# surrealdb/surrealdb

Measured on AMD Instinct MI355X. Metric: knn_qps, higher is better.
Workload: dtype f32; 1 GPU; brute-force cosine KNN, 10000000 rows/GPU x 768-dim f32, K=10, single query (BASELINE configs[1]); batch=0, rows_total=10000000, rows_per_gpu=10000000, dim=768, k=10, distance=cosine, parallelism=single

## Files before the change

surrealdb_amd/csrc/sdbv.hip:

```cpp

#include <hip/hip_runtime.h>
#include <rocblas/rocblas.h>

#include <algorithm>
#include <atomic>
#include <cfloat>
#include <chrono>
#include <cmath>
#include <cstdint>
#include <deque>
#include <limits>
#include <memory>
#include <thread>
#include <unordered_set>
#include <cstdio>
#include <cstring>
#include <map>
#include <mutex>
#include <queue>
#include <set>
#include <string>
#include <unordered_map>
#include <vector>

// ... 17 lines not shown
struct Shadow {
	int kind = 0;
	bool h4 = false;
	void *codes = nullptr;
	float *side = nullptr;
	uint64_t sn_pad = 0;
	uint64_t bytes = 0;
	float *pinv() const { return side; }
	float *pscale() const { return side; }
	float *peps() const { return side + sn_pad; }
	float *l2_xx() const { return side + sn_pad; }
	float *l2_res() const { return side + 2 * sn_pad; }
	uint32_t *xsum() const { return (uint32_t *)(side + 2 * sn_pad); }
	float *peps4() const { return h4 ? side + 3 * sn_pad : nullptr; }
	uint32_t *xsum_h() const {
		return h4 ? (uint32_t *)(side + 4 * sn_pad) : nullptr;
	}
	uint32_t *plane_h() const { return (uint32_t *)codes; }
	uint32_t *plane_l(uint32_t d) const {
		return plane_h() + (uint64_t)((d + 31) / 32) * sn_pad * 4;
	}
};

struct Table {
	uint64_t n = 0;
	uint64_t n_pad = 0;
	uint32_t d = 0;
	uint8_t metric = 0;
	double order = 0.0;
	float *cm = nullptr;
	double *norms = nullptr;
	float *aux = nullptr;
	uint32_t *bunc = nullptr;
	uint32_t bunc_n = 0;
	double bmax_norm = 0.0;
	uint64_t *ids_dev = nullptr;
	Shadow sh;
	uint64_t bytes = 0;
};

struct sdbv_ctx {
	int device = 0;
	hipStream_t stream = nullptr;
	std::map<uint64_t, Table> tables;
	std::mutex mu;
	std::string err;
	sdbv_stats stats{};
	void *block_out = nullptr;
	uint64_t block_out_cap = 0;
	void *final_out = nullptr;
	void *merge_tmp = nullptr;
	float *q_dev = nullptr;
	float *q_pin = nullptr;
	uint32_t q_cap = 0;
	hipEvent_t ev0, ev1, ev2, ev3, ev4;
	float *pf_scores = nullptr;
	uint64_t pf_scores_cap = 0;
	uint32_t *pf_rows = nullptr;
	uint32_t *pf4_list = nullptr;
	void *pf4_thr = nullptr;
	void *pf_cands = nullptr;
	void *pf_res = nullptr;
	uint64_t pf_slots[2][6] = {};
	rocblas_handle blas = nullptr;
	float *S = nullptr;
	uint64_t S_cap = 0;
	void *bstate = nullptr;
	uint64_t bstate_cap = 0;
	float *Q_dev = nullptr;
	uint64_t Q_cap = 0;
	double *qnorms = nullptr;
	uint64_t qnorms_cap = 0;
	double *bdists = nullptr;
	uint64_t bdists_cap = 0;
	uint32_t *btheta = nullptr;
	uint64_t btheta_cap = 0;
	void *bcand = nullptr;
	uint64_t bcand_cap = 0;
	uint32_t *bcand_cnt = nullptr;
	uint64_t bcand_cnt_cap = 0;
	double ms_gemm = 0, ms_select = 0, ms_exact = 0;
	uint64_t *flt_mask = nullptr;
	uint64_t *flt_mask_pin = nullptr;
	uint64_t flt_mask_cap = 0;
	uint32_t *flt_rows = nullptr;
	uint32_t *flt_rows_pin = nullptr;
	void *flt_cands = nullptr;
};

struct Cand {
	double dist;
	uint64_t id;
};

__device__ __host__ static inline uint64_t d_splitmix64(uint64_t z) {
	z += 0x9E3779B97F4A7C15ULL;
	z = (z ^ (z >> 30)) * 0xBF58476D1CE4E5B9ULL;
	z = (z ^ (z >> 27)) * 0x94D049BB133111EBULL;
	return z ^ (z >> 31);
}

__device__ __host__ static inline float d_gen_elem(uint64_t seed, uint64_t gidx) {
	uint64_t x = d_splitmix64(seed + gidx);
	double u = (double)(x >> 11) * 0x1.0p-53;
	return (float)(-20.0 + 40.0 * u);
}

__device__ static inline uint64_t d_total_key(double x) {
	uint64_t bits = __double_as_longlong(x);
	return (bits >> 63) ? ~bits : (bits | 0x8000000000000000ULL);
}


__global__ void k_gen_cm(float *cm, uint64_t n, uint64_t n_pad, uint32_t d,
                         uint64_t seed, uint64_t row_offset) {
	uint64_t total = (uint64_t)d * n_pad;
	for (uint64_t idx = (uint64_t)blockIdx.x * blockDim.x + threadIdx.x;
	     idx < total; idx += (uint64_t)gridDim.x * blockDim.x) {
		uint64_t k = idx / n_pad;
		uint64_t r = idx % n_pad;
		float v = 0.0f;
		if (r < n)
			v = d_gen_elem(seed, (row_offset + r) * (uint64_t)d + k);
		cm[idx] = v;
	}
}

__global__ void k_transpose(const float *__restrict__ rm, float *__restrict__ cm,
                            uint64_t n, uint64_t n_pad, uint32_t d) {
	__shared__ float tile[32][33];
	uint64_t rb = (uint64_t)blockIdx.x * 32;
	uint32_t kb = blockIdx.y * 32;
	uint32_t tx = threadIdx.x & 31, ty = threadIdx.x >> 5;
	for (uint32_t yy = ty; yy < 32; yy += 8) {
		uint64_t r = rb + yy;
		uint32_t k = kb + tx;
		tile[yy][tx] = (r < n && k < d) ? rm[r * d + k] : 0.0f;
	}
	__syncthreads();
	for (uint32_t yy = ty; yy < 32; yy += 8) {
		uint32_t k = kb + yy;
		uint64_t r = rb + tx;
		if (k < d && r < n_pad)
			cm[(uint64_t)k * n_pad + r] = tile[tx][yy];
	}
}

__global__ void k_norms(const float *__restrict__ cm, double *__restrict__ norms,
                        uint64_t n, uint64_t n_pad, uint32_t d) {
	uint64_t r = (uint64_t)blockIdx.x * blockDim.x + threadIdx.x;
	if (r >= n)
		return;
	float p[8] = {0, 0, 0, 0, 0, 0, 0, 0};
	uint32_t k = 0;
	for (; k + 8 <= d; k += 8) {
#pragma unroll
		for (uint32_t j = 0; j < 8; j++) {
			float x = cm[(uint64_t)(k + j) * n_pad + r];
			p[j] = __fadd_rn(p[j], __fmul_rn(x, x));
		}
	}
	float acc = 0.0f;
	acc = __fadd_rn(acc, __fadd_rn(__fadd_rn(p[0], p[4]), __fadd_rn(p[1], p[5])));
// ... 204 lines not shown
					acc.y = __fadd_rn(acc.y, __fmul_rn(dy, dy));
					acc.z = __fadd_rn(acc.z, __fmul_rn(dz, dz));
					acc.w = __fadd_rn(acc.w, __fmul_rn(dw, dw));
				}
				const float s[4] = {acc.x, acc.y, acc.z, acc.w};
#pragma unroll
				for (int c = 0; c < ROWS_PER_LANE; c++)
					dist[c] = sqrt((double)s[c]);
			}
		}

		uint64_t kk_key = kth_key;
		uint32_t kk_row = kth_row;
		int full = (topk_n >= (int)k);
#pragma unroll
		for (int c = 0; c < ROWS_PER_LANE; c++) {
			if (!valid[c])
				continue;
			uint64_t key = d_total_key(dist[c]);
			uint32_t row32 = (uint32_t)(r0 + c);
			bool take = !full || key < kk_key || (key == kk_key && row32 < kk_row);
			if (take) {
				int idx = atomicAdd(&cnt, 1);
				buf[idx].key = key;
				buf[idx].dist = dist[c];
				buf[idx].row = row32;
			}
		}
		__syncthreads();

		if (cnt > 0) {
			int m = cnt;
			for (int i = threadIdx.x; i < topk_n; i += THREADS)
				buf[m + i] = topk[i];
			int total = m + topk_n;
			__syncthreads();
			int new_n;
			block_select_topk(buf, total, topk, (int)k, &new_n);
			if (threadIdx.x == 0) {
				topk_n = new_n;
				if (new_n >= (int)k) {
					kth_key = topk[k - 1].key;
					kth_row = topk[k - 1].row;
				}
				cnt = 0;
			}
		}
		__syncthreads();
	}

	scan_topk_write(topk, topk_n, k, ids, block_out);
}

__device__ __forceinline__ static void merge_slice(
    Cand *__restrict__ block_out, uint64_t total, uint32_t k,
    uint64_t per_block, Cand *__restrict__ out) {
	__shared__ uint64_t red_key[THREADS / 64];
	__shared__ uint64_t red_id[THREADS / 64];
	__shared__ long red_idx[THREADS / 64];
	const int lane = threadIdx.x & 63;
	const int wave = threadIdx.x >> 6;
	const uint64_t s0 = (uint64_t)blockIdx.x * per_block;
	const uint64_t s1 = s0 + per_block < total ? s0 + per_block : total;
	out += (uint64_t)blockIdx.x * k;
	if (s0 >= total) {
		for (uint32_t i = threadIdx.x; i < k; i += THREADS) {
			out[i].dist = __longlong_as_double(0x7FF0000000000000LL);
			out[i].id = ~0ULL;
		}
		return;
	}
	for (int slot = 0; slot < (int)k; slot++) {
		uint64_t bk = ~0ULL;
		uint64_t bid = ~0ULL;
		long bi = -1;
		for (uint64_t i = s0 + threadIdx.x; i < s1; i += THREADS) {
			uint64_t ck = d_total_key(block_out[i].dist);
			uint64_t cid = block_out[i].id;
			if (ck < bk || (ck == bk && cid < bid)) {
				bk = ck;
				bid = cid;
				bi = (long)i;
			}
		}
		for (int off = 32; off > 0; off >>= 1) {
			uint64_t ok = __shfl_down(bk, off);
			uint64_t oid = __shfl_down(bid, off);
			long oi = __shfl_down(bi, off);
			if (ok < bk || (ok == bk && oid < bid)) {
				bk = ok;
				bid = oid;
				bi = oi;
			}
		}
		if (lane == 0) {
			red_key[wave] = bk;
			red_id[wave] = bid;
			red_idx[wave] = bi;
		}
		__syncthreads();
		if (threadIdx.x == 0) {
			uint64_t bbk = ~0ULL, bbid = ~0ULL;
			long best = -1;
			for (int w = 0; w < THREADS / 64; w++) {
				if (red_idx[w] < 0)
					continue;
				if (red_key[w] < bbk ||
				    (red_key[w] == bbk && red_id[w] < bbid)) {
					bbk = red_key[w];
					bbid = red_id[w];
					best = red_idx[w];
				}
			}
			if (best < 0) {
				out[slot].dist =
				    __longlong_as_double(0x7FF0000000000000LL);
				out[slot].id = ~0ULL;
			} else {
				out[slot] = block_out[best];
				block_out[best].dist =
				    __longlong_as_double(0x7FF0000000000000LL);
				block_out[best].id = ~0ULL;
// ... 881 lines not shown
			const int32_t N =
			    H4 ? (int32_t)(8u * (256u * ah2 + 16u * ah1 + ah0) -
			                   16384u * xsum[r] + qbias)
			       : PF6_N(xsum[r], qbias);
			const float pe = peps[r];
			const float a = PF6_A(
			    N, H4 ? __fmul_rn(pscale[r], 0.5f) : pscale[r], qscale);
			const float e = PF6_E(pe, qeps);
			const bool ok = allowed && r < row_end &&
			                (__float_as_uint(a) & 0x7F800000u) != 0x7F800000u;
			if constexpr (MASKED)
				scores[r] = ok        ? __fsub_rn(a, e)
				            : allowed ? ninf
				                      : __uint_as_float(0x7FC00000u);
			else
				scores[r] = ok ? __fsub_rn(a, e) : ninf;
			if (ok) {
				const uint64_t v =
				    ((uint64_t)d_key32(__fadd_rn(a, e)) << 32) | (uint32_t)r;
				if (!full || v < kthv) {
					int idx = atomicAdd(&cnt, 1);
					buf[idx] = v;
				}
			}
		}
		pf_topk_fold(buf, topk, cnt, topk_n, kth, k);
	}

	pf_topk_write(topk, topk_n, k, block_out);
}

__global__ void k_pf_compact(const float *__restrict__ scores, uint64_t n,
                             const Cand *__restrict__ approx_top, uint32_t k,
                             float eps, uint32_t *__restrict__ cand_cnt,
                             uint32_t *__restrict__ cand_rows) {
	const double thr = approx_top[k - 1].dist + 2.0 * (double)eps;
	const uint64_t ngrp = (n + 3) / 4;
	for (uint64_t g = (uint64_t)blockIdx.x * blockDim.x + threadIdx.x;
	     g < ngrp; g += (uint64_t)gridDim.x * blockDim.x) {
		const float4 s = *(const float4 *)(scores + g * 4);
		const float v[4] = {s.x, s.y, s.z, s.w};
#pragma unroll
		for (int c = 0; c < 4; c++) {
			uint64_t r = g * 4 + c;
			if (r < n && (double)v[c] <= thr) {
				uint32_t idx = atomicAdd(cand_cnt, 1u);
				if (idx < PF_CAND_CAP)
					cand_rows[idx] = (uint32_t)r;
			}
		}
	}
}

template <int METRIC>
__device__ __forceinline__ static void rows_exact_one(
    const float *__restrict__ cm, const double *__restrict__ norms,
    const uint64_t *__restrict__ ids, uint64_t n_pad, uint32_t d,
    double q_norm, uint32_t r, Cand *__restrict__ out, float *qs, float *xs,
    float *ps) {
	__syncthreads();
	for (uint32_t i = threadIdx.x; i < d; i += 64)
		xs[i] = cm[(uint64_t)i * n_pad + r];
	__syncthreads();
	if (METRIC == 0) {
		const uint32_t d8 = d & ~7u;
		if (threadIdx.x < 8) {
			float pj = 0.f;
			for (uint32_t i = threadIdx.x; i < d8; i += 8)
				pj = __fadd_rn(pj, __fmul_rn(xs[i], qs[i]));
			ps[threadIdx.x] = pj;
		}
		__syncthreads();
		if (threadIdx.x == 0) {
			float p[8];
#pragma unroll
			for (int j = 0; j < 8; j++)
				p[j] = ps[j];
			uint32_t k8 = d8;
			float sum = 0.f;
			sum = __fadd_rn(sum, __fadd_rn(p[0], p[4]));
			sum = __fadd_rn(sum, __fadd_rn(p[1], p[5]));
			sum = __fadd_rn(sum, __fadd_rn(p[2], p[6]));
			sum = __fadd_rn(sum, __fadd_rn(p[3], p[7]));
			for (; k8 < d; k8++)
				sum = __fadd_rn(sum, __fmul_rn(xs[k8], qs[k8]));
			double den = q_norm * norms[r];
			Cand o;
			o.dist = 1.0 - (double)sum / den;
			o.id = ids[r];
			*out = o;
		}
	} else {
		if (threadIdx.x == 0) {
			float acc = 0.f;
			for (uint32_t kk = 0; kk < d; kk++) {
				float diff = xs[kk] - qs[kk];
				acc = __fadd_rn(acc, __fmul_rn(diff, diff));
			}
			Cand o;
			o.dist = sqrt((double)acc);
			o.id = ids[r];
			*out = o;
		}
	}
}

template <int METRIC>
__device__ __forceinline__ static void rows_exact(
    const float *__restrict__ cm, const double *__restrict__ norms,
    const uint64_t *__restrict__ ids, uint64_t n_pad, uint32_t d,
    const float *__restrict__ qg, double q_norm,
    const uint32_t *__restrict__ rows, uint32_t cnt, Cand *__restrict__ out,
    float *qs, float *xs, float *ps) {
	for (uint32_t i = threadIdx.x; i < d; i += 64)
		qs[i] = qg[i];
	for (uint32_t c = blockIdx.x; c < cnt; c += gridDim.x)
		rows_exact_one<METRIC>(cm, norms, ids, n_pad, d, q_norm, rows[c],
		                       out + c, qs, xs, ps);
}

template <int METRIC>
__global__ __launch_bounds__(64) void k_pf_rescore(
    const float *__restrict__ cm, const double *__restrict__ norms,
    const uint64_t *__restrict__ ids, uint64_t n_pad, uint32_t d,
    const float *__restrict__ qg, double q_norm,
    const uint32_t *__restrict__ cand_cnt,
    const uint32_t *__restrict__ cand_rows, Cand *__restrict__ out) {
	__shared__ float qs[MAX_D];
	__shared__ float xs[MAX_D];
	__shared__ float ps[8];
	const uint32_t cnt = *cand_cnt;
	if (cnt > PF_CAND_CAP || blockIdx.x >= cnt)
		return;
	rows_exact<METRIC>(cm, norms, ids, n_pad, d, qg, q_norm, cand_rows, cnt,
	                   out, qs, xs, ps);
}

template <int METRIC>
__global__ __launch_bounds__(64) void k_rows_exact(
    const float *__restrict__ cm, const double *__restrict__ norms,
    const uint64_t *__restrict__ ids, uint64_t n_pad, uint32_t d,
    const float *__restrict__ qg, double q_norm,
    const uint32_t *__restrict__ rows, uint32_t cnt, Cand *__restrict__ out) {
	__shared__ float qs[MAX_D];
	__shared__ float xs[MAX_D];
	__shared__ float ps[8];
	rows_exact<METRIC>(cm, norms, ids, n_pad, d, qg, q_norm, rows, cnt, out,
	                   qs, xs, ps);
}

__global__ __launch_bounds__(THREADS) void k_pf_final(
    Cand *__restrict__ cands, const uint32_t *__restrict__ cand_cnt,
    uint32_t k, Cand *__restrict__ out) {
	const uint32_t raw = *cand_cnt;
	const uint64_t total = raw > PF_CAND_CAP ? 0 : raw;
	if (threadIdx.x == 0) {
		out[k].dist = 0.0;
		out[k].id = raw;
	}
	merge_slice(cands, total, k, total, out);
}

#define PF4_LIST_CAP 262144u
#define PF4_BLOCK_LIST 8192
#define PF4_PASSES 4
#ifndef PF4_REFINE_LANES
#define PF4_REFINE_LANES 32
#endif

__global__ __launch_bounds__(64) void k_pf4_threshold(
    const float *__restrict__ cm, const double *__restrict__ norms,
    const uint64_t *__restrict__ ids, uint64_t n_pad, uint32_t d,
    const float *__restrict__ qg, double q_norm,
    const Cand *__restrict__ approx_top, Cand *__restrict__ out) {
	__shared__ float qs[MAX_D];
	__shared__ float xs[MAX_D];
	__shared__ float ps[8];
	const uint64_t r = approx_top[blockIdx.x].id;
	if (r == ~0ULL) {
		if (threadIdx.x == 0) {
			Cand o;
			o.dist = __longlong_as_double(0x7FF0000000000000LL);
			o.id = ~0ULL;
			out[blockIdx.x] = o;
		}
		return;
	}
	for (uint32_t i = threadIdx.x; i < d; i += 64)
		qs[i] = qg[i];
	rows_exact_one<0>(cm, norms, ids, n_pad, d, q_norm, (uint32_t)r,
	                  out + blockIdx.x, qs, xs, ps);
}

__device__ __forceinline__ static double pf4_threshold(
    const Cand *__restrict__ thr, uint32_t k, unsigned long long *key) {
	if (threadIdx.x == 0)
		*key = 0;
	__syncthreads();
	if (threadIdx.x < k)
		atomicMax(key, (unsigned long long)d_total_key(thr[threadIdx.x].dist));
	__syncthreads();
	const uint64_t kb = *key;
	return __longlong_as_double(
	    (long long)((kb >> 63) ? (kb & 0x7FFFFFFFFFFFFFFFULL) : ~kb));
}

__global__ __launch_bounds__(THREADS) void k_pf4_compact(
    const float *__restrict__ scores, uint64_t n,
    const Cand *__restrict__ thr, uint32_t k, uint32_t list_cap,
    uint32_t *__restrict__ list_cnt, uint32_t *__restrict__ list_rows) {
	__shared__ uint32_t rows[PF4_BLOCK_LIST];
	__shared__ uint32_t cnt, base;
	__shared__ unsigned long long tkey;
	if (threadIdx.x == 0)
		cnt = 0;
	const double T = pf4_threshold(thr, k, &tkey);
	const uint64_t ngrp = (n + 3) / 4;
	const uint64_t round = (uint64_t)THREADS * PF4_PASSES;
	for (uint64_t g0 = (uint64_t)blockIdx.x * round;;
	     g0 += (uint64_t)gridDim.x * round) {
		const bool last = g0 >= ngrp;
		float4 s[PF4_PASSES];
#pragma unroll
		for (int p = 0; p < PF4_PASSES; p++) {
			const uint64_t g = g0 + (uint64_t)p * THREADS + threadIdx.x;
			if (g < ngrp)
				s[p] = *(const float4 *)(scores + g * 4);
		}
#pragma unroll
		for (int p = 0; p < PF4_PASSES; p++) {
			const uint64_t g = g0 + (uint64_t)p * THREADS + threadIdx.x;
			if (g >= ngrp)
				continue;
			const float v[4] = {s[p].x, s[p].y, s[p].z, s[p].w};
#pragma unroll
			for (int c = 0; c < 4; c++) {
				const uint64_t r = g * 4 + c;
				if (r < n && !((double)v[c] > T))
					rows[atomicAdd(&cnt, 1u)] = (uint32_t)r;
			}
		}
		__syncthreads();
		const uint32_t m = cnt;
		__syncthreads();
		if (m > PF4_BLOCK_LIST - 4 * THREADS * PF4_PASSES || (last && m > 0)) {
			if (threadIdx.x == 0) {
				base = atomicAdd(list_cnt, m);
				cnt = 0;
			}
			__syncthreads();
			for (uint32_t i = threadIdx.x; i < m; i += THREADS)
				if (base + i < list_cap)
					list_rows[base + i] = rows[i];
			__syncthreads();
		}
		if (last)
			break;
	}
}

__global__ __launch_bounds__(THREADS) void k_pf4_refine(
    const uint4 *__restrict__ hp, const uint2 *__restrict__ lp,
    const float *__restrict__ pscale, const float *__restrict__ peps,
    const uint32_t *__restrict__ xsum, uint64_t sn_pad, uint32_t ngroups,
    const uint32_t *__restrict__ qd, float qscale, float qeps, uint32_t qbias,
    const Cand *__restrict__ thr, uint32_t k, uint32_t list_cap,
    const uint32_t *__restrict__ list_cnt,
    const uint32_t *__restrict__ list_rows, uint32_t *__restrict__ cand_cnt,
    uint32_t *__restrict__ cand_rows) {
	__shared__ unsigned long long tkey;
	const double T = pf4_threshold(thr, k, &tkey);
	const uint32_t m = *list_cnt;
	if (m > list_cap)
		return;
	const uint32_t sub = threadIdx.x % PF4_REFINE_LANES;
	const uint32_t per_grid = gridDim.x * (THREADS / PF4_REFINE_LANES);
	for (uint32_t c = (blockIdx.x * THREADS + threadIdx.x) / PF4_REFINE_LANES;
	     c < m; c += per_grid) {
		const uint32_t r = list_rows[c];
		uint32_t ah2 = 0, ah1 = 0, ah0 = 0, al2 = 0, al1 = 0, al0 = 0;
		for (uint32_t g = sub; g < ngroups; g += PF4_REFINE_LANES) {
			const uint4 hv = hp[(uint64_t)g * sn_pad + r];
			const uint2 lv = lp[(uint64_t)g * sn_pad + r];
			PF6_GROUP(hv, lv, g)
		}
#pragma unroll
		for (int off = PF4_REFINE_LANES / 2; off > 0; off >>= 1) {
			ah2 += __shfl_xor(ah2, off);
			ah1 += __shfl_xor(ah1, off);
			ah0 += __shfl_xor(ah0, off);
			al2 += __shfl_xor(al2, off);
			al1 += __shfl_xor(al1, off);
			al0 += __shfl_xor(al0, off);
		}
		if (sub == 0) {
			const int32_t N = PF6_N(xsum[r], qbias);
			const float pe = peps[r];
			const float a = PF6_A(N, pscale[r], qscale);
			const float e = PF6_E(pe, qeps);
			const bool covered =
			    (__float_as_uint(a) & 0x7F800000u) != 0x7F800000u;
			if (!covered || !((double)__fsub_rn(a, e) > T)) {
				const uint32_t idx = atomicAdd(cand_cnt, 1u);
				if (idx < PF_CAND_CAP)
					cand_rows[idx] = r;
			}
		}
	}
}
#undef PF6_E
#undef PF6_A
#undef PF6_N
#undef PF6_GROUP
#undef PF6_GROUP_H
#undef PF6_DOT3

template <int METRIC>
__global__ void k_all_dists(const float *__restrict__ cm,
                            const double *__restrict__ norms, uint64_t n,
                            uint64_t n_pad, uint32_t d,
                            const float *__restrict__ qg, double q_norm,
                            double order, double q_mean,
                            double *__restrict__ out) {
	uint64_t r = (uint64_t)blockIdx.x * blockDim.x + threadIdx.x;
	if (r >= n)
		return;
	if (METRIC == 0) {
		float p[8] = {0, 0, 0, 0, 0, 0, 0, 0};
		uint32_t k = 0;
		for (; k + 8 <= d; k += 8) {
#pragma unroll
			for (uint32_t j = 0; j < 8; j++) {
				float x = cm[(uint64_t)(k + j) * n_pad + r];
				p[j] = __fadd_rn(p[j], __fmul_rn(x, qg[k + j]));
			}
		}
		float sum = 0.f;
		sum = __fadd_rn(sum, __fadd_rn(p[0], p[4]));
		sum = __fadd_rn(sum, __fadd_rn(p[1], p[5]));
		sum = __fadd_rn(sum, __fadd_rn(p[2], p[6]));
		sum = __fadd_rn(sum, __fadd_rn(p[3], p[7]));
		for (; k < d; k++)
			sum = __fadd_rn(sum, __fmul_rn(cm[(uint64_t)k * n_pad + r], qg[k]));
		out[r] = 1.0 - (double)sum / (q_norm * norms[r]);
	} else if (METRIC == 1) {
		float acc = 0.f;
		for (uint32_t k = 0; k < d; k++) {
			float diff = cm[(uint64_t)k * n_pad + r] - qg[k];
			acc = __fadd_rn(acc, __fmul_rn(diff, diff));
		}
		out[r] = sqrt((double)acc);
	} else if (METRIC == 2) {
		float acc = 0.f;
		for (uint32_t k = 0; k < d; k++)
			acc = __fadd_rn(acc, fabsf(qg[k] - cm[(uint64_t)k * n_pad + r]));
		out[r] = (double)acc;
	} else if (METRIC == 3) {
		float m = 0.f;
		for (uint32_t k = 0; k < d; k++)
			m = fmaxf(m, fabsf(qg[k] - cm[(uint64_t)k * n_pad + r]));
// ... 1093 lines not shown
		(void)hipFree(t.norms);
	if (t.aux)
		(void)hipFree(t.aux);
	if (t.bunc)
		(void)hipFree(t.bunc);
	if (t.ids_dev)
		(void)hipFree(t.ids_dev);
	if (t.sh.codes)
		(void)hipFree(t.sh.codes);
	if (t.sh.side)
		(void)hipFree(t.sh.side);
	t = Table{};
}

extern "C" {

int sdbv_init(int device, sdbv_ctx **out) {
	auto *ctx = new sdbv_ctx();
	if (device >= 0) {
		if (hipSetDevice(device) != hipSuccess) {
			delete ctx;
			return SDBV_ERR_HIP;
		}
		ctx->device = device;
	} else {
		(void)hipGetDevice(&ctx->device);
	}
	if (hipStreamCreate(&ctx->stream) != hipSuccess) {
		delete ctx;
		return SDBV_ERR_HIP;
	}
	(void)hipEventCreate(&ctx->ev0);
	(void)hipEventCreate(&ctx->ev1);
	(void)hipEventCreate(&ctx->ev2);
	(void)hipEventCreate(&ctx->ev3);
	(void)hipEventCreate(&ctx->ev4);
	*out = ctx;
	return SDBV_OK;
}

void sdbv_shutdown(sdbv_ctx *ctx) {
	if (!ctx)
		return;
	for (auto &kv : ctx->tables)
		free_table(kv.second);
	if (ctx->block_out)
		(void)hipFree(ctx->block_out);
	if (ctx->final_out)
		(void)hipFree(ctx->final_out);
	if (ctx->merge_tmp)
		(void)hipFree(ctx->merge_tmp);
	if (ctx->q_dev)
		(void)hipFree(ctx->q_dev);
	for (void *p : {(void *)ctx->pf_scores, (void *)ctx->pf_rows,
	                ctx->pf_cands, ctx->pf_res, (void *)ctx->pf4_list,
	                ctx->pf4_thr})
		if (p)
			(void)hipFree(p);
	for (void *p : {(void *)ctx->S, ctx->bstate, (void *)ctx->Q_dev,
	                (void *)ctx->qnorms, (void *)ctx->bdists,
	                (void *)ctx->btheta, (void *)ctx->bcand,
	                (void *)ctx->bcand_cnt})
		if (p)
			(void)hipFree(p);
	for (void *p : {(void *)ctx->flt_mask, (void *)ctx->flt_rows,
	                ctx->flt_cands})
		if (p)
			(void)hipFree(p);
	if (ctx->flt_mask_pin)
		(void)hipHostFree(ctx->flt_mask_pin);
	if (ctx->flt_rows_pin)
		(void)hipHostFree(ctx->flt_rows_pin);
	if (ctx->blas)
		(void)rocblas_destroy_handle(ctx->blas);
	(void)hipEventDestroy(ctx->ev0);
	(void)hipEventDestroy(ctx->ev1);
	(void)hipEventDestroy(ctx->ev2);
	(void)hipEventDestroy(ctx->ev3);
	(void)hipEventDestroy(ctx->ev4);
	(void)hipStreamDestroy(ctx->stream);
	delete ctx;
}

const char *sdbv_last_error(sdbv_ctx *ctx) { return ctx ? ctx->err.c_str() : ""; }

int sdbv_get_stats(sdbv_ctx *ctx, sdbv_stats *out) {
	if (!ctx || !out)
		return SDBV_ERR_BAD_ARG;
	*out = ctx->stats;
	return SDBV_OK;
}

static int stage_common(sdbv_ctx *ctx, uint64_t table, uint64_t n, uint32_t d,
                        uint8_t metric, Table **out) {
	if (d == 0 || d > MAX_D || (d % 4) != 0)
		return SDBV_ERR_BAD_ARG;
	if (metric > SDBV_METRIC_PEARSON)
		return SDBV_ERR_UNSUPPORTED;
	if (metric == SDBV_METRIC_JACCARD && d > 1024)
		return SDBV_ERR_UNSUPPORTED;
	auto it = ctx->tables.find(table);
	if (it != ctx->tables.end()) {
		free_table(it->second);
		ctx->tables.erase(it);
	}
	Table t;
// ... 413 lines not shown
	hipLaunchKernelGGL(k_fill_ids, dim3((uint32_t)nb), dim3(THREADS), 0,
	                   ctx->stream, t->ids_dev, t->n_pad, id_base);
	return finish_stage(ctx, t, true);
}

uint64_t sdbv_table_rows(sdbv_ctx *ctx, uint64_t table) {
	std::lock_guard<std::mutex> lk(ctx->mu);
	auto it = ctx->tables.find(table);
	return it == ctx->tables.end() ? 0 : it->second.n;
}

int sdbv_drop_table(sdbv_ctx *ctx, uint64_t table) {
	std::lock_guard<std::mutex> lk(ctx->mu);
	auto it = ctx->tables.find(table);
	if (it == ctx->tables.end())
		return SDBV_ERR_NO_TABLE;
	free_table(it->second);
	ctx->tables.erase(it);
	refresh_bytes_staged(ctx);
	return SDBV_OK;
}

int sdbv_table_set_order(sdbv_ctx *ctx, uint64_t table, double order) {
	std::lock_guard<std::mutex> lk(ctx->mu);
	auto it = ctx->tables.find(table);
	if (it == ctx->tables.end())
		return SDBV_ERR_NO_TABLE;
	it->second.order = order;
	return SDBV_OK;
}

static int ensure_query_scratch(sdbv_ctx *ctx, uint32_t d, uint64_t nblocks,
                                uint32_t k) {
	if (ctx->q_cap < d) {
		if (ctx->q_dev)
			(void)hipFree(ctx->q_dev);
		const size_t qb = d * sizeof(float) +
		                  (size_t)((d + 31) / 32) * PF6_QWORDS * sizeof(uint32_t);
		HIP_CHECK(ctx, hipMalloc(&ctx->q_dev, qb));
		if (ctx->q_pin)
			(void)hipHostFree(ctx->q_pin);
		HIP_CHECK(ctx, hipHostMalloc(&ctx->q_pin, qb));
		ctx->q_cap = d;
	}
	uint64_t need = nblocks * k * sizeof(Cand);
	if (ctx->block_out_cap < need) {
		if (ctx->block_out)
			(void)hipFree(ctx->block_out);
		HIP_CHECK(ctx, hipMalloc(&ctx->block_out, need));
		ctx->block_out_cap = need;
	}
	if (!ctx->final_out)
		HIP_CHECK(ctx, hipMalloc(&ctx->final_out, MAX_K * sizeof(Cand)));
	if (!ctx->merge_tmp)
		HIP_CHECK(ctx,
		          hipMalloc(&ctx->merge_tmp, 32 * MAX_K * sizeof(Cand)));
	return SDBV_OK;
}

static int stage_query(sdbv_ctx *ctx, const float *q, uint32_t d,
                       size_t q_bytes) {
	std::memcpy(ctx->q_pin, q, d * sizeof(float));
	HIP_CHECK(ctx, hipMemcpyAsync(ctx->q_dev, ctx->q_pin, q_bytes,
	                              hipMemcpyHostToDevice, ctx->stream));
	return SDBV_OK;
}

static void copy_results(const Cand *host_out, uint32_t m, uint64_t *out_ids,
                         double *out_dists, uint32_t *out_n) {
	*out_n = m;
	for (uint32_t i = 0; i < m; i++) {
		out_ids[i] = host_out[i].id;
		out_dists[i] = host_out[i].dist;
	}
}

static uint64_t scan_grid(uint64_t n, uint64_t *rows_per_block) {
	uint64_t tiles = (n + TILE - 1) / TILE;
	uint64_t nblocks = tiles < 2048 ? tiles : 2048;
	if (nblocks == 0)
		nblocks = 1;
	uint64_t tiles_per_block = (tiles + nblocks - 1) / nblocks;
	*rows_per_block = tiles_per_block * TILE;
	return (n + *rows_per_block - 1) / *rows_per_block;
}

static void launch_scan(sdbv_ctx *ctx, Table &t, uint32_t k, double q_norm,
                        uint64_t nblocks, uint64_t rows_per_block,
                        const uint64_t *mask) {
#define LAUNCH_SCAN(M, MASKED)                                                 \
	hipLaunchKernelGGL((k_scan<M, MASKED>), dim3((uint32_t)nblocks),           \
	                   dim3(THREADS), 0, ctx->stream, t.cm, t.norms, t.n,      \
	                   t.n_pad, t.d, ctx->q_dev, q_norm, k, rows_per_block,    \
	                   (Cand *)ctx->block_out, t.ids_dev, mask)
	const bool cosine = t.metric == SDBV_METRIC_COSINE;
	if (mask) {
		if (cosine)
			LAUNCH_SCAN(0, true);
		else
			LAUNCH_SCAN(1, true);
	} else {
		if (cosine)
			LAUNCH_SCAN(0, false);
		else
			LAUNCH_SCAN(1, false);
	}
// ... 430 lines not shown
	ctx->stats.last_scan_kernel_ms = ms_scan;
	ctx->stats.last_merge_kernel_ms = ms_merge;
	ctx->stats.last_rows_scanned = t.n;
	return SDBV_OK;
}

int sdbv_knn_bruteforce(sdbv_ctx *ctx, uint64_t table, const float *q,
                        uint32_t d, uint32_t k, uint64_t *out_ids,
                        double *out_dists, uint32_t *out_n) {
	std::lock_guard<std::mutex> lk(ctx->mu);
	auto it = ctx->tables.find(table);
	if (it == ctx->tables.end())
		return SDBV_ERR_NO_TABLE;
	Table &t = it->second;
	if (d != t.d)
		return SDBV_ERR_BAD_ARG;
	if (k == 0 || k > (1u << 22))
		return SDBV_ERR_BAD_ARG;
	ctx->stats.last_scan_path = 0;
	ctx->stats.last_prefilter_candidates = 0;
	ctx->stats.last_prefilter_stage1 = 0;
	if (k > MAX_K || t.metric > SDBV_METRIC_EUCLIDEAN)
		return knn_large_k(ctx, t, q, d, k, nullptr, out_ids, out_dists,
		                   out_n);

	uint64_t rows_per_block = 0;
	const uint64_t nblocks = scan_grid(t.n, &rows_per_block);
	const int kind = shadow_kind(t);
	const bool use_h4 = kind == 3 && t.sh.h4 && h4_policy(&t);
	uint64_t pf_rows_per_block = 0;
	uint64_t scratch_blocks = std::max(
	    nblocks,
	    kind ? prefilter_grid(ctx, t.n, kind, false, &pf_rows_per_block) : 0);
	if (use_h4)
		scratch_blocks = std::max(
		    scratch_blocks,
		    prefilter_grid(ctx, t.n, 4, false, &pf_rows_per_block));
	int rc = ensure_query_scratch(ctx, d, scratch_blocks, k);
	if (rc != SDBV_OK)
		return rc;
	double q_norm = sqrt((double)h_sumsq_f32(q, d));
	PfL2Q l2q;
	const bool use_pf =
	    kind == 5 ? pf_l2_query(q, d, &l2q)
	              : kind != 0 && q_norm >= PF_NORM_MIN && q_norm <= PF_NORM_MAX;
	PfQ6 q6;
	float qbias = 0.f;
	rc = stage_query_pf(ctx, q, d, q_norm, use_pf ? kind : 0, &q6, &qbias,
	                    &l2q);
	if (rc != SDBV_OK)
		return rc;

	auto t_start = std::chrono::steady_clock::now();
	Cand host_out[MAX_K + 2];
	bool served = false;
	if (use_pf && use_h4) {
		const uint32_t list_cap = pf4_list_max();
		uint32_t ncand = 0, nstage1 = 0;
		rc = knn_prefilter_h4(ctx, t, k, q_norm, q6, list_cap, host_out,
		                      &ncand, &nstage1);
		if (rc != SDBV_OK)
			return rc;
		ctx->stats.last_prefilter_stage1 = nstage1;
		if (nstage1 <= list_cap) {
			served = true;
			ctx->stats.last_prefilter_candidates = ncand;
			ctx->stats.last_scan_path = ncand <= PF_CAND_CAP ? 15u : 16u;
		}
	}
	if (use_pf && !served) {
		uint32_t ncand = 0;
		rc = knn_prefilter(ctx, t, k, q_norm, qbias, q6, nullptr, host_out,
		                   &ncand);
		if (rc != SDBV_OK)
			return rc;
		ctx->stats.last_prefilter_candidates = ncand;
		ctx->stats.last_scan_path = (ncand <= PF_CAND_CAP ? 1u : 2u) +
		                            (kind == 5 ? 16u : 2u * (uint32_t)(kind - 1));
	}
	if (!(ctx->stats.last_scan_path & 1u)) {
		rc = knn_exact_scan(ctx, t, k, q_norm, nblocks, rows_per_block,
		                    host_out);
		if (rc != SDBV_OK)
			return rc;
	}
	ctx->stats.last_total_ms =
	    std::chrono::duration<double, std::milli>(
	        std::chrono::steady_clock::now() - t_start)
	        .count();

	copy_results(host_out, (uint32_t)(k < t.n ? k : t.n), out_ids, out_dists,
	             out_n);
	return SDBV_OK;
}


uint64_t sdbv_filter_rows(const uint64_t *allow, uint64_t allow_words,
                          uint64_t n, uint32_t *out_rows, uint64_t cap) {
	if (!allow)
		return 0;
	uint64_t words = (n + 63) / 64;
	if (words > allow_words)
		words = allow_words;
	if (!out_rows)
		cap = 0;
	uint64_t count = 0;
	for (uint64_t w = 0; w < words; w++) {
// ... 122 lines not shown
	if (!allow || allow_words != (t.n + 63) / 64)
		return SDBV_ERR_BAD_ARG;
	auto t_start = std::chrono::steady_clock::now();
	const bool device_topk = k <= MAX_K && t.metric <= SDBV_METRIC_EUCLIDEAN;
	const uint64_t list_max = device_topk ? filter_rowlist_max() : 0;
	if (list_max && !ctx->flt_rows_pin)
		HIP_CHECK(ctx, hipHostMalloc(&ctx->flt_rows_pin,
		                             PF_CAND_CAP * sizeof(uint32_t)));
	const uint64_t count = sdbv_filter_rows(allow, allow_words, t.n,
	                                        ctx->flt_rows_pin, list_max);
	ctx->stats.last_scan_path = 0;
	ctx->stats.last_prefilter_candidates = 0;
	ctx->stats.last_prefilter_stage1 = 0;
	ctx->stats.last_filter_rows = count;
	ctx->stats.last_rows_scanned = count;
	ctx->stats.last_scan_kernel_ms = 0;
	ctx->stats.last_merge_kernel_ms = 0;
	ctx->stats.last_total_ms = 0;
	if (count == 0) {
		*out_n = 0;
		return SDBV_OK;
	}
	if (!device_topk)
		return knn_large_k(ctx, t, q, d, k, allow, out_ids, out_dists, out_n);

	const bool by_list = count <= list_max;
	double q_norm = sqrt((double)h_sumsq_f32(q, d));
	const int kind = shadow_kind(t);
	PfL2Q l2q;
	const bool use_pf =
	    !by_list && kind != 0 && filter_prefilter_policy(t) &&
	    (kind == 5 ? pf_l2_query(q, d, &l2q)
	               : q_norm >= PF_NORM_MIN && q_norm <= PF_NORM_MAX);
	uint64_t rows_per_block = 0;
	const uint64_t nblocks = scan_grid(t.n, &rows_per_block);
	uint64_t pf_rows_per_block = 0;
	const uint64_t scratch_blocks = std::max(
	    nblocks,
	    use_pf ? prefilter_grid(ctx, t.n, kind, true, &pf_rows_per_block) : 0);
	int rc = ensure_query_scratch(ctx, d, by_list ? 1 : scratch_blocks, k);
	if (rc != SDBV_OK)
		return rc;
	PfQ6 q6;
	float qbias = 0.f;
	rc = stage_query_pf(ctx, q, d, q_norm, use_pf ? kind : 0, &q6, &qbias,
	                    &l2q);
	if (rc != SDBV_OK)
		return rc;
	if (!by_list) {
		rc = upload_filter_mask(ctx, t, allow, allow_words);
		if (rc != SDBV_OK)
			return rc;
	}
	Cand host_out[MAX_K + 1];
	if (use_pf) {
		uint32_t ncand = 0;
		rc = knn_prefilter(ctx, t, k, q_norm, qbias, q6, ctx->flt_mask,
		                   host_out, &ncand);
		if (rc != SDBV_OK)
			return rc;
		ctx->stats.last_prefilter_candidates = ncand;
		ctx->stats.last_scan_path = (ncand <= PF_CAND_CAP ? 9u : 10u) +
		                            (kind == 5 ? 10u : 2u * (uint32_t)(kind - 1));
	}
	if (!(ctx->stats.last_scan_path & 1u)) {
		if (by_list)
			rc = knn_row_list(ctx, t, k, q_norm, (uint32_t)count, host_out);
		else
			rc = knn_masked_scan(ctx, t, k, q_norm, nblocks, rows_per_block,
			                     host_out);
		if (rc != SDBV_OK)
			return rc;
		float ms_scan = 0, ms_merge = 0;
		(void)hipEventElapsedTime(&ms_scan, ctx->ev0, ctx->ev1);
		(void)hipEventElapsedTime(&ms_merge, ctx->ev1, ctx->ev2);
		ctx->stats.last_scan_kernel_ms = ms_scan;
		ctx->stats.last_merge_kernel_ms = ms_merge;
		if (!use_pf)
			ctx->stats.last_scan_path = by_list ? 8u : 7u;
	}
	ctx->stats.last_total_ms =
	    std::chrono::duration<double, std::milli>(
	        std::chrono::steady_clock::now() - t_start)
	        .count();

	copy_results(host_out, (uint32_t)(k < count ? k : count), out_ids,
	             out_dists, out_n);
	return SDBV_OK;
}

int sdbv_all_distances(sdbv_ctx *ctx, uint64_t table, const float *q,
                       uint32_t d, double *out) {
	std::lock_guard<std::mutex> lk(ctx->mu);
	auto it = ctx->tables.find(table);
	if (it == ctx->tables.end())
		return SDBV_ERR_NO_TABLE;
	Table &t = it->second;
	if (d != t.d)
		return SDBV_ERR_BAD_ARG;
	int rc = ensure_query_scratch(ctx, d, 1, 1);
	if (rc != SDBV_OK)
		return rc;
	std::memcpy(ctx->q_pin, q, d * sizeof(float));
	HIP_CHECK(ctx, hipMemcpyAsync(ctx->q_dev, ctx->q_pin, d * sizeof(float),
	                              hipMemcpyHostToDevice, ctx->stream));
	double *dout = nullptr;
	HIP_CHECK(ctx, hipMalloc(&dout, t.n * sizeof(double)));
// ... 300 lines not shown
		for (int c = 0; c < kk; c++) {
			BCand bc = h_state[(uint64_t)j * kk + c];
			if (bc.row == ~0u)
				continue;
			double dd = h_dists[(uint64_t)j * kk + c];
			cand[m++] = {{total_key(dd), ids_host[bc.row]}, dd};
			bkey = std::max(bkey, bc.key);
		}
		std::sort(cand.begin(), cand.begin() + m);
		if (m == (size_t)kk) {
			const double dk = cand[k - 1].second, qn = h_qnorm[j];
			const double ek = t.metric == SDBV_METRIC_COSINE
			                      ? -((1.0 - dk) * qn)
			                      : dk * dk - qn * qn;
			const double bound =
			    sdbv_batch_key_bound(t.metric, d, qn, t.bmax_norm);
			if (!((double)bkey > ek + bound)) {
				to_exact[j] = 1;
				continue;
			}
		}
		for (uint32_t c = 0; c < n_unc; c++) {
			double dd = h_unc_dists[(uint64_t)j * n_unc + c];
			cand[m++] = {{total_key(dd), ids_host[h_unc[c]]}, dd};
		}
		if (n_unc)
			std::sort(cand.begin(), cand.begin() + m);
		uint32_t out_m = (uint32_t)std::min<size_t>(k, m);
		for (uint32_t c = 0; c < out_m; c++) {
			out_ids[(uint64_t)j * k + c] = cand[c].first.second;
			out_dists[(uint64_t)j * k + c] = cand[c].second;
		}
		for (uint32_t c = out_m; c < k; c++) {
			out_ids[(uint64_t)j * k + c] = ~0ULL;
			out_dists[(uint64_t)j * k + c] =
			    std::numeric_limits<double>::infinity();
		}
	}

	uint64_t rows_per_block = 0;
	const uint64_t nblocks = scan_grid(t.n, &rows_per_block);
	bool scratch_ready = false;
	for (uint32_t j = 0; j < b; j++) {
		if (!to_exact[j])
			continue;
		if (!scratch_ready) {
			if ((rc = ensure_query_scratch(ctx, d, nblocks, k)))
				return rc;
			scratch_ready = true;
		}
		const float *q = Q + (uint64_t)j * d;
		if ((rc = stage_query(ctx, q, d, d * sizeof(float))))
			return rc;
		Cand host_out[MAX_K];
		if ((rc = knn_exact_scan(ctx, t, k, h_qnorm[j], nblocks, rows_per_block,
		                         host_out)))
			return rc;
		const uint32_t out_m = (uint32_t)std::min<uint64_t>(k, t.n);
		for (uint32_t c = 0; c < out_m; c++) {
			out_ids[(uint64_t)j * k + c] = host_out[c].id;
			out_dists[(uint64_t)j * k + c] = host_out[c].dist;
		}
		for (uint32_t c = out_m; c < k; c++) {
			out_ids[(uint64_t)j * k + c] = ~0ULL;
			out_dists[(uint64_t)j * k + c] =
			    std::numeric_limits<double>::infinity();
		}
		ctx->stats.last_batch_exact_queries++;
	}
	ctx->ms_gemm = ms_gemm;
	ctx->ms_select = ms_select;
	ctx->ms_exact = me;
	ctx->stats.last_scan_kernel_ms = ms_gemm;
	ctx->stats.last_merge_kernel_ms = ms_select;
	ctx->stats.last_rows_scanned = t.n;
	return SDBV_OK;
}
}


namespace hnsw {

static inline uint64_t total_key(double x) {
	uint64_t bits;
	std::memcpy(&bits, &x, 8);
	return (bits >> 63) ? ~bits : (bits | 0x8000000000000000ULL);
}

struct PQ {
	struct E {
		uint64_t key;
		uint32_t seq;
		uint32_t id;
		double d;
	};
	std::vector<E> v;
	size_t head = 0;
	uint32_t next_seq = 0;
	size_t n = 0;
	void push(double d, uint32_t id) {
		E e{total_key(d), next_seq++, id, d};
		auto it = std::upper_bound(
		    v.begin() + head, v.end(), e, [](const E &a, const E &b) {
			    return a.key != b.key ? a.key < b.key : a.seq < b.seq;
		    });
		v.insert(it, e);
		n++;
// ... 3958 lines not shown
```

Before: 1273 queries/s.

## Add rank-based fast merge, prefetch rescore/compact loads, pin result buffers

Several latency-focused tweaks for the single-query path. Small candidate sets (up to 512) are now merged with a rank-based selection in shared memory instead of k sequential argmin passes. The rescore and refine kernels issue their row loads before the threshold reduction and prefetch the next candidate row. The compact kernel double-buffers its score loads. Query staging is folded into the first row load, and host results go to pinned memory so readback avoids pageable copies. The risks are extra register pressure and more complex tie-breaking logic in the merge.

```diff
diff --git a/surrealdb_amd/csrc/sdbv.hip b/surrealdb_amd/csrc/sdbv.hip
--- a/surrealdb_amd/csrc/sdbv.hip
+++ b/surrealdb_amd/csrc/sdbv.hip
@@ -93,6 +93,7 @@
 	void *merge_tmp = nullptr;
 	float *q_dev = nullptr;
 	float *q_pin = nullptr;
+	void *res_pin = nullptr;
 	uint32_t q_cap = 0;
 	hipEvent_t ev0, ev1, ev2, ev3, ev4;
 	float *pf_scores = nullptr;
@@ -150,6 +151,11 @@
 __device__ static inline uint64_t d_total_key(double x) {
 	uint64_t bits = __double_as_longlong(x);
 	return (bits >> 63) ? ~bits : (bits | 0x8000000000000000ULL);
+}
+
+__device__ static inline double d_key_dist(uint64_t key) {
+	return __longlong_as_double(
+	    (long long)((key >> 63) ? (key & 0x7FFFFFFFFFFFFFFFULL) : ~key));
 }
 
 
@@ -460,6 +466,108 @@
 	scan_topk_write(topk, topk_n, k, ids, block_out);
 }
 
+#define MERGE_FAST_MAX 512u
+#define MERGE_KEY_INF 0xFFF0000000000000ULL
+
+#define MERGE_E (MERGE_FAST_MAX / THREADS)
+
+__device__ __forceinline__ static void merge_ranked_load(
+    const Cand *__restrict__ src, uint32_t readable, uint64_t *mk,
+    uint64_t *mid) {
+	const uint32_t lane = threadIdx.x & 63;
+	const uint32_t wave = threadIdx.x >> 6;
+#pragma unroll
+	for (uint32_t t = 0; t < MERGE_E; t++) {
+		const uint32_t p = (THREADS / 64) * (64 * t + lane) + wave;
+		const Cand c = src[p < readable ? p : 0];
+		mk[t] = d_total_key(c.dist);
+		mid[t] = c.id;
+	}
+}
+
+__device__ __forceinline__ static uint32_t merge_rank(
+    const ulonglong2 *list, uint32_t n, uint64_t mk, uint64_t mid,
+    uint32_t mypos) {
+	uint32_t mh = (uint32_t)(mk >> 32);
+	asm volatile("" : "+v"(mh));
+	n = __builtin_amdgcn_readfirstlane(n);
+	uint32_t r = 0;
+	for (uint32_t j = 0; j < n; j += 4) {
+		ulonglong2 o[4];
+#pragma unroll
+		for (uint32_t jj = 0; jj < 4; jj++)
+			o[jj] = list[j + jj];
+#pragma unroll
+		for (uint32_t jj = 0; jj < 4; jj++) {
+			uint32_t oh = (uint32_t)(o[jj].x >> 32);
+			asm volatile("" : "+v"(oh));
+			r += (uint32_t)(oh < mh);
+			const uint32_t tie =
+			    (uint32_t)(oh == mh) & (uint32_t)(j + jj != mypos);
+			if (__any(tie))
+				r += tie &
+				     ((uint32_t)(o[jj].x < mk) |
+				      ((uint32_t)(o[jj].x == mk) &
+				       ((uint32_t)(o[jj].y < mid) |
+				        ((uint32_t)(o[jj].y == mid) &
+				         (uint32_t)(j + jj < mypos)))));
+		}
+	}
+	return r;
+}
+
+__device__ __forceinline__ static void merge_ranked_select(
+    uint64_t *mk, uint64_t *mid, uint32_t len, uint32_t k,
+    Cand *__restrict__ out) {
+	constexpr uint32_t WAVES = THREADS / 64;
+	static_assert(WAVES * MAX_K == THREADS, "one thread per handed-on entry");
+	static_assert(WAVES % 4 == 0, "the second ranking reads by fours");
+	__shared__ ulonglong2 ent[MERGE_FAST_MAX];
+	__shared__ ulonglong2 win[WAVES * MAX_K];
+	const uint32_t lane = threadIdx.x & 63;
+	const uint32_t wave = threadIdx.x >> 6;
+	ulonglong2 *we = ent + wave * 64 * MERGE_E;
+	const uint32_t cw = len > wave ? (len - wave + WAVES - 1) / WAVES : 0;
+#pragma unroll
+	for (uint32_t t = 0; t < MERGE_E; t++) {
+		if (64 * t + lane >= cw) {
+			mk[t] = ~0ULL;
+			mid[t] = ~0ULL;
+		}
+		we[64 * t + lane] = make_ulonglong2(mk[t], mid[t]);
+	}
+	if (threadIdx.x < WAVES * k)
+		win[threadIdx.x] = make_ulonglong2(~0ULL, ~0ULL);
+	__syncthreads();
+#pragma unroll
+	for (uint32_t t = 0; t < MERGE_E; t++) {
+		if (64 * t >= cw)
+			break;
+		const uint32_t r =
+		    merge_rank(we, cw, mk[t], mid[t], 64 * t + lane);
+		if (64 * t + lane < cw && r < k)
+			win[wave * k + r] = make_ulonglong2(mk[t], mid[t]);
+	}
+	__syncthreads();
+	const uint32_t nw = WAVES * k;
+	if (threadIdx.x < nw) {
+		const ulonglong2 my = win[threadIdx.x];
+		const uint32_t r = merge_rank(win, nw, my.x, my.y, threadIdx.x);
+		if (r < k) {
+			const bool some = my.x != ~0ULL || my.y != ~0ULL;
+			Cand c;
+			if (some && (r == 0 || my.x <= MERGE_KEY_INF)) {
+				c.dist = d_key_dist(my.x);
+				c.id = my.y;
+			} else {
+				c.dist = __longlong_as_double(0x7FF0000000000000LL);
+				c.id = ~0ULL;
+			}
+			out[r] = c;
+		}
+	}
+}
+
 __device__ __forceinline__ static void merge_slice(
     Cand *__restrict__ block_out, uint64_t total, uint32_t k,
     uint64_t per_block, Cand *__restrict__ out) {
@@ -476,6 +584,12 @@
 			out[i].dist = __longlong_as_double(0x7FF0000000000000LL);
 			out[i].id = ~0ULL;
 		}
+		return;
+	}
+	if (s1 - s0 <= MERGE_FAST_MAX) {
+		uint64_t mk[MERGE_E], mid[MERGE_E];
+		merge_ranked_load(block_out + s0, (uint32_t)(s1 - s0), mk, mid);
+		merge_ranked_select(mk, mid, (uint32_t)(s1 - s0), k, out);
 		return;
 	}
 	for (int slot = 0; slot < (int)k; slot++) {
@@ -1463,22 +1577,61 @@
 	}
 }
 
+#define ROWS_EXACT_FLY 16
+#define ROWS_SUM_FLY 16
 template <int METRIC>
 __device__ __forceinline__ static void rows_exact_one(
     const float *__restrict__ cm, const double *__restrict__ norms,
     const uint64_t *__restrict__ ids, uint64_t n_pad, uint32_t d,
     double q_norm, uint32_t r, Cand *__restrict__ out, float *qs, float *xs,
-    float *ps) {
+    float *ps, const float *__restrict__ qg) {
+	double norm_r = 0.0;
+	if (METRIC == 0)
+		norm_r = norms[r];
+	const uint64_t id_r = ids[r];
 	__syncthreads();
-	for (uint32_t i = threadIdx.x; i < d; i += 64)
-		xs[i] = cm[(uint64_t)i * n_pad + r];
+	for (uint32_t b0 = 0; b0 < d; b0 += 64 * ROWS_EXACT_FLY) {
+		const uint32_t i0 = b0 + threadIdx.x;
+		float v[ROWS_EXACT_FLY];
+#pragma unroll
+		for (uint32_t u = 0; u < ROWS_EXACT_FLY; u++)
+			if (i0 + 64 * u < d)
+				v[u] = cm[(uint64_t)(i0 + 64 * u) * n_pad + r];
+		if (qg) {
+			for (uint32_t i = threadIdx.x; i < d; i += 64)
+				qs[i] = qg[i];
+			qg = nullptr;
+			__syncthreads();
+		}
+#pragma unroll
+		for (uint32_t u = 0; u < ROWS_EXACT_FLY; u++)
+			if (i0 + 64 * u < d) {
+				const float qk = qs[i0 + 64 * u];
+				if (METRIC == 0) {
+					xs[i0 + 64 * u] = __fmul_rn(v[u], qk);
+				} else {
+					const float diff = v[u] - qk;
+					xs[i0 + 64 * u] = __fmul_rn(diff, diff);
+				}
+			}
+	}
 	__syncthreads();
 	if (METRIC == 0) {
 		const uint32_t d8 = d & ~7u;
 		if (threadIdx.x < 8) {
 			float pj = 0.f;
-			for (uint32_t i = threadIdx.x; i < d8; i += 8)
-				pj = __fadd_rn(pj, __fmul_rn(xs[i], qs[i]));
+			uint32_t i = threadIdx.x;
+			for (; i + 8 * (ROWS_SUM_FLY - 1) < d8; i += 8 * ROWS_SUM_FLY) {
+				float t[ROWS_SUM_FLY];
+#pragma unroll
+				for (uint32_t u = 0; u < ROWS_SUM_FLY; u++)
+					t[u] = xs[i + 8 * u];
+#pragma unroll
+				for (uint32_t u = 0; u < ROWS_SUM_FLY; u++)
+					pj = __fadd_rn(pj, t[u]);
+			}
+			for (; i < d8; i += 8)
+				pj = __fadd_rn(pj, xs[i]);
 			ps[threadIdx.x] = pj;
 		}
 		__syncthreads();
@@ -1494,23 +1647,31 @@
 			sum = __fadd_rn(sum, __fadd_rn(p[2], p[6]));
 			sum = __fadd_rn(sum, __fadd_rn(p[3], p[7]));
 			for (; k8 < d; k8++)
-				sum = __fadd_rn(sum, __fmul_rn(xs[k8], qs[k8]));
-			double den = q_norm * norms[r];
+				sum = __fadd_rn(sum, xs[k8]);
+			double den = q_norm * norm_r;
 			Cand o;
 			o.dist = 1.0 - (double)sum / den;
-			o.id = ids[r];
+			o.id = id_r;
 			*out = o;
 		}
 	} else {
 		if (threadIdx.x == 0) {
 			float acc = 0.f;
-			for (uint32_t kk = 0; kk < d; kk++) {
-				float diff = xs[kk] - qs[kk];
-				acc = __fadd_rn(acc, __fmul_rn(diff, diff));
-			}
+			uint32_t kk = 0;
+			for (; kk + ROWS_SUM_FLY <= d; kk += ROWS_SUM_FLY) {
+				float t[ROWS_SUM_FLY];
+#pragma unroll
+				for (uint32_t u = 0; u < ROWS_SUM_FLY; u++)
+					t[u] = xs[kk + u];
+#pragma unroll
+				for (uint32_t u = 0; u < ROWS_SUM_FLY; u++)
+					acc = __fadd_rn(acc, t[u]);
+			}
+			for (; kk < d; kk++)
+				acc = __fadd_rn(acc, xs[kk]);
 			Cand o;
 			o.dist = sqrt((double)acc);
-			o.id = ids[r];
+			o.id = id_r;
 			*out = o;
 		}
 	}
@@ -1521,13 +1682,16 @@
     const float *__restrict__ cm, const double *__restrict__ norms,
     const uint64_t *__restrict__ ids, uint64_t n_pad, uint32_t d,
     const float *__restrict__ qg, double q_norm,
-    const uint32_t *__restrict__ rows, uint32_t cnt, Cand *__restrict__ out,
-    float *qs, float *xs, float *ps) {
-	for (uint32_t i = threadIdx.x; i < d; i += 64)
-		qs[i] = qg[i];
-	for (uint32_t c = blockIdx.x; c < cnt; c += gridDim.x)
-		rows_exact_one<METRIC>(cm, norms, ids, n_pad, d, q_norm, rows[c],
-		                       out + c, qs, xs, ps);
+    const uint32_t *__restrict__ rows, uint32_t r_first, uint32_t cnt,
+    Cand *__restrict__ out, float *qs, float *xs, float *ps) {
+	uint32_t r = r_first;
+	for (uint32_t c = blockIdx.x; c < cnt; c += gridDim.x) {
+		const uint32_t cn = c + gridDim.x;
+		const uint32_t rn = cn < cnt ? rows[cn] : 0;
+		rows_exact_one<METRIC>(cm, norms, ids, n_pad, d, q_norm, r, out + c,
+		                       qs, xs, ps, c == blockIdx.x ? qg : nullptr);
+		r = rn;
+	}
 }
 
 template <int METRIC>
@@ -1540,11 +1704,13 @@
 	__shared__ float qs[MAX_D];
 	__shared__ float xs[MAX_D];
 	__shared__ float ps[8];
+	static_assert(PF_RESCORE_BLOCKS <= PF_CAND_CAP, "r_first is in the list");
 	const uint32_t cnt = *cand_cnt;
+	const uint32_t r_first = cand_rows[blockIdx.x];
 	if (cnt > PF_CAND_CAP || blockIdx.x >= cnt)
 		return;
-	rows_exact<METRIC>(cm, norms, ids, n_pad, d, qg, q_norm, cand_rows, cnt,
-	                   out, qs, xs, ps);
+	rows_exact<METRIC>(cm, norms, ids, n_pad, d, qg, q_norm, cand_rows,
+	                   r_first, cnt, out, qs, xs, ps);
 }
 
 template <int METRIC>
@@ -1556,20 +1722,27 @@
 	__shared__ float qs[MAX_D];
 	__shared__ float xs[MAX_D];
 	__shared__ float ps[8];
-	rows_exact<METRIC>(cm, norms, ids, n_pad, d, qg, q_norm, rows, cnt, out,
-	                   qs, xs, ps);
+	const uint32_t r_first = blockIdx.x < cnt ? rows[blockIdx.x] : 0;
+	rows_exact<METRIC>(cm, norms, ids, n_pad, d, qg, q_norm, rows, r_first,
+	                   cnt, out, qs, xs, ps);
 }
 
 __global__ __launch_bounds__(THREADS) void k_pf_final(
     Cand *__restrict__ cands, const uint32_t *__restrict__ cand_cnt,
     uint32_t k, Cand *__restrict__ out) {
+	static_assert(MERGE_FAST_MAX <= PF_CAND_CAP, "the list has these slots");
 	const uint32_t raw = *cand_cnt;
+	uint64_t mk[MERGE_E], mid[MERGE_E];
+	merge_ranked_load(cands, MERGE_FAST_MAX, mk, mid);
 	const uint64_t total = raw > PF_CAND_CAP ? 0 : raw;
 	if (threadIdx.x == 0) {
 		out[k].dist = 0.0;
 		out[k].id = raw;
 	}
-	merge_slice(cands, total, k, total, out);
+	if (total >= 1 && total <= MERGE_FAST_MAX)
+		merge_ranked_select(mk, mid, (uint32_t)total, k, out);
+	else
+		merge_slice(cands, total, k, total, out);
 }
 
 #define PF4_LIST_CAP 262144u
@@ -1597,10 +1770,8 @@
 		}
 		return;
 	}
-	for (uint32_t i = threadIdx.x; i < d; i += 64)
-		qs[i] = qg[i];
 	rows_exact_one<0>(cm, norms, ids, n_pad, d, q_norm, (uint32_t)r,
-	                  out + blockIdx.x, qs, xs, ps);
+	                  out + blockIdx.x, qs, xs, ps, qg);
 }
 
 __device__ __forceinline__ static double pf4_threshold(
@@ -1611,9 +1782,7 @@
 	if (threadIdx.x < k)
 		atomicMax(key, (unsigned long long)d_total_key(thr[threadIdx.x].dist));
 	__syncthreads();
-	const uint64_t kb = *key;
-	return __longlong_as_double(
-	    (long long)((kb >> 63) ? (kb & 0x7FFFFFFFFFFFFFFFULL) : ~kb));
+	return d_key_dist(*key);
 }
 
 __global__ __launch_bounds__(THREADS) void k_pf4_compact(
@@ -1625,18 +1794,27 @@
 	__shared__ unsigned long long tkey;
 	if (threadIdx.x == 0)
 		cnt = 0;
-	const double T = pf4_threshold(thr, k, &tkey);
 	const uint64_t ngrp = (n + 3) / 4;
 	const uint64_t round = (uint64_t)THREADS * PF4_PASSES;
-	for (uint64_t g0 = (uint64_t)blockIdx.x * round;;
-	     g0 += (uint64_t)gridDim.x * round) {
+	uint64_t g0 = (uint64_t)blockIdx.x * round;
+	float4 s[PF4_PASSES], sn[PF4_PASSES];
+#pragma unroll
+	for (int p = 0; p < PF4_PASSES; p++) {
+		const uint64_t g = g0 + (uint64_t)p * THREADS + threadIdx.x;
+		s[p] = make_float4(0.f, 0.f, 0.f, 0.f);
+		if (g < ngrp)
+			s[p] = *(const float4 *)(scores + g * 4);
+	}
+	const double T = pf4_threshold(thr, k, &tkey);
+	for (;; g0 += (uint64_t)gridDim.x * round) {
 		const bool last = g0 >= ngrp;
-		float4 s[PF4_PASSES];
 #pragma unroll
 		for (int p = 0; p < PF4_PASSES; p++) {
-			const uint64_t g = g0 + (uint64_t)p * THREADS + threadIdx.x;
+			const uint64_t g = g0 + (uint64_t)gridDim.x * round +
+			                   (uint64_t)p * THREADS + threadIdx.x;
+			sn[p] = make_float4(0.f, 0.f, 0.f, 0.f);
 			if (g < ngrp)
-				s[p] = *(const float4 *)(scores + g * 4);
+				sn[p] = *(const float4 *)(scores + g * 4);
 		}
 #pragma unroll
 		for (int p = 0; p < PF4_PASSES; p++) {
@@ -1667,6 +1845,9 @@
 		}
 		if (last)
 			break;
+#pragma unroll
+		for (int p = 0; p < PF4_PASSES; p++)
+			s[p] = sn[p];
 	}
 }
 
@@ -1680,21 +1861,30 @@
     const uint32_t *__restrict__ list_rows, uint32_t *__restrict__ cand_cnt,
     uint32_t *__restrict__ cand_rows) {
 	__shared__ unsigned long long tkey;
+	const uint32_t sub = threadIdx.x % PF4_REFINE_LANES;
+	const uint32_t per_grid = gridDim.x * (THREADS / PF4_REFINE_LANES);
+	uint32_t c = (blockIdx.x * THREADS + threadIdx.x) / PF4_REFINE_LANES;
+	const uint32_t m = *list_cnt;
+	uint32_t r = c < PF4_LIST_CAP ? list_rows[c] : 0;
 	const double T = pf4_threshold(thr, k, &tkey);
-	const uint32_t m = *list_cnt;
 	if (m > list_cap)
 		return;
-	const uint32_t sub = threadIdx.x % PF4_REFINE_LANES;
-	const uint32_t per_grid = gridDim.x * (THREADS / PF4_REFINE_LANES);
-	for (uint32_t c = (blockIdx.x * THREADS + threadIdx.x) / PF4_REFINE_LANES;
-	     c < m; c += per_grid) {
-		const uint32_t r = list_rows[c];
+	for (; c < m; c += per_grid) {
+		uint32_t xs_r = 0;
+		float pe = 0.f, ps_r = 0.f;
+		if (sub == 0) {
+			xs_r = xsum[r];
+			pe = peps[r];
+			ps_r = pscale[r];
+		}
 		uint32_t ah2 = 0, ah1 = 0, ah0 = 0, al2 = 0, al1 = 0, al0 = 0;
 		for (uint32_t g = sub; g < ngroups; g += PF4_REFINE_LANES) {
 			const uint4 hv = hp[(uint64_t)g * sn_pad + r];
 			const uint2 lv = lp[(uint64_t)g * sn_pad + r];
 			PF6_GROUP(hv, lv, g)
 		}
+		const uint32_t cn = c + per_grid;
+		const uint32_t r_next = cn < m ? list_rows[cn] : 0;
 #pragma unroll
 		for (int off = PF4_REFINE_LANES / 2; off > 0; off >>= 1) {
 			ah2 += __shfl_xor(ah2, off);
@@ -1705,9 +1895,8 @@
 			al0 += __shfl_xor(al0, off);
 		}
 		if (sub == 0) {
-			const int32_t N = PF6_N(xsum[r], qbias);
-			const float pe = peps[r];
-			const float a = PF6_A(N, pscale[r], qscale);
+			const int32_t N = PF6_N(xs_r, qbias);
+			const float a = PF6_A(N, ps_r, qscale);
 			const float e = PF6_E(pe, qeps);
 			const bool covered =
 			    (__float_as_uint(a) & 0x7F800000u) != 0x7F800000u;
@@ -1717,6 +1906,7 @@
 					cand_rows[idx] = r;
 			}
 		}
+		r = r_next;
 	}
 }
 #undef PF6_E
@@ -2916,6 +3106,10 @@
 		(void)hipFree(ctx->merge_tmp);
 	if (ctx->q_dev)
 		(void)hipFree(ctx->q_dev);
+	if (ctx->q_pin)
+		(void)hipHostFree(ctx->q_pin);
+	if (ctx->res_pin)
+		(void)hipHostFree(ctx->res_pin);
 	for (void *p : {(void *)ctx->pf_scores, (void *)ctx->pf_rows,
 	                ctx->pf_cands, ctx->pf_res, (void *)ctx->pf4_list,
 	                ctx->pf4_thr})
@@ -3435,6 +3629,9 @@
 	}
 	if (!ctx->final_out)
 		HIP_CHECK(ctx, hipMalloc(&ctx->final_out, MAX_K * sizeof(Cand)));
+	if (!ctx->res_pin)
+		HIP_CHECK(ctx,
+		          hipHostMalloc(&ctx->res_pin, (MAX_K + 2) * sizeof(Cand)));
 	if (!ctx->merge_tmp)
 		HIP_CHECK(ctx,
 		          hipMalloc(&ctx->merge_tmp, 32 * MAX_K * sizeof(Cand)));
@@ -3971,7 +4168,7 @@
 		return rc;
 
 	auto t_start = std::chrono::steady_clock::now();
-	Cand host_out[MAX_K + 2];
+	Cand *host_out = (Cand *)ctx->res_pin;
 	bool served = false;
 	if (use_pf && use_h4) {
 		const uint32_t list_cap = pf4_list_max();
@@ -4200,7 +4397,7 @@
 		if (rc != SDBV_OK)
 			return rc;
 	}
-	Cand host_out[MAX_K + 1];
+	Cand *host_out = (Cand *)ctx->res_pin;
 	if (use_pf) {
 		uint32_t ncand = 0;
 		rc = knn_prefilter(ctx, t, k, q_norm, qbias, q6, ctx->flt_mask,
@@ -4607,7 +4804,7 @@
 		const float *q = Q + (uint64_t)j * d;
 		if ((rc = stage_query(ctx, q, d, d * sizeof(float))))
 			return rc;
-		Cand host_out[MAX_K];
+		Cand *host_out = (Cand *)ctx->res_pin;
 		if ((rc = knn_exact_scan(ctx, t, k, h_qnorm[j], nblocks, rows_per_block,
 		                         host_out)))
 			return rc;
```

Measured after the change: 1232 queries/s. -3.2%, worse.
